# caishiqing/voice-tts

Measured on AMD Instinct MI355X. Metric: audio_seconds_per_second, higher is better.
Workload: dtype bf16

## Files before the change

include/ixtts_hip.h:

```cpp
#ifndef IXTTS_HIP_H
#define IXTTS_HIP_H

#include <stddef.h>
#include <stdint.h>

#ifdef __cplusplus
extern "C" {
#endif

#define IXTTS_OK 0
#define IXTTS_ERR_ARG (-1)
#define IXTTS_ERR_HIP (-2)
#define IXTTS_ERR_STATE (-3)
#define IXTTS_ERR_NOMEM (-4)
#define IXTTS_ERR_NAME (-5)

const char* ixtts_version(void);
const char* ixtts_last_error(void);

int ixtts_aa_snake_f32(const float* x_dev, float* y_dev, const float* up12_dev, const float* down12_dev,
                       const float* log_alpha_dev, const float* log_beta_dev, int B, int C, int T, void* stream);

size_t ixtts_attn_full_workspace_bytes(int B, int H, int T);
int ixtts_attn_full_f32(const float* q_dev, const float* k_dev, const float* v_dev, float* out_dev, int B, int H, int T,
// ... 18 lines not shown
int ixtts_adaln_rmsnorm_varlen_f32(const float* x_dev, const float* wb_dev, const float* g_dev, float* out_dev, const int* seq_off_dev, int nseq,
                                   long rows, int H, float eps, void* stream);
int ixtts_ln_modulate_varlen_f32(const float* x_dev, const float* shift_scale_dev, float* out_dev, const int* seq_off_dev, int nseq, long rows, int H,
                                 float eps, void* stream);
int ixtts_rope_qk_varlen_f32(float* qkv_dev, const float* cos_sin_dev, const int* seq_off_dev, int nseq, long rows, int H, int head_dim, void* stream);
int ixtts_wn_gate_rows_varlen_f32(const float* a_dev, const float* g_dev, float* out_dev, long rows, int C, const int* seq_off_dev, int nseq,
                                  long g_stride, int g_offset, void* stream);
int ixtts_reflect_halo_rows_varlen_f32(float* p_dev, const int* seq_off_dev, int nseq, int C, int left, int right, void* stream);

size_t ixtts_gemm_x6_packed_bytes(int N, int K);
int ixtts_gemm_x6_pack(const float* w_dev, void* packed_dev, int N, int K, void* stream);
long ixtts_gemm_x6_rows_padded(long rows);
int ixtts_gemm_x6_split(const float* a_dev, long lda, void* planes_dev, long rows, int K, void* stream);
int ixtts_gemm_x6_f32(const void* a_planes_dev, long rows_total, long row0, const void* packed_dev, const float* bias_dev, float* c_dev, long ldc,
                      int M, int N, int K, int accumulate, int tile, void* stream);
int ixtts_gemm_x6_pair_f32(const void* a_planes_dev, long rows_total, long row0, int taps, const void* packed_dev, const float* bias_dev,
                           const float* gate_dev, long gate_ld, long rows_per_batch, int nbatch, float* c_dev, long ldc, int M, int N, int K,
                           int epilogue, int tile, void* stream);
int ixtts_gemm_x6_pair_gate_varlen_f32(const void* a_planes_dev, long rows_total, long row0, int taps, const void* packed_dev, const float* bias_dev,
                                       const float* gate_dev, long gate_ld, const int* seq_off_dev, int nseq, float* c_dev, long ldc, int M, int N,
                                       int K, int tile, void* stream);

#define IXTTS_BIGVGAN_MAX_STAGES 8
#define IXTTS_BIGVGAN_MAX_RESK 4

typedef struct ixtts_bigvgan_cfg {
  int num_mels;
  int upsample_initial_channel;
  int n_stages;
  int upsample_rates[IXTTS_BIGVGAN_MAX_STAGES];
  int upsample_kernel_sizes[IXTTS_BIGVGAN_MAX_STAGES];
  int n_resblock_kernels;
  int resblock_kernel_sizes[IXTTS_BIGVGAN_MAX_RESK];
  int resblock_dilations[IXTTS_BIGVGAN_MAX_RESK][3];
  int max_frames;
  int fast_sin;
// ... 132 lines not shown
```

voice-tts_amd/_lib.py:

```python
import ctypes as C
import os

HERE = os.path.dirname(os.path.abspath(__file__))
LIB_PATH = os.environ.get("IXTTS_LIB") or os.path.join(HERE, "libixtts_hip.so")

MAX_STAGES = 8
MAX_RESK = 4


class BigVGANCfg(C.Structure):
    _fields_ = [
        ("num_mels", C.c_int), ("upsample_initial_channel", C.c_int), ("n_stages", C.c_int),
        ("upsample_rates", C.c_int * MAX_STAGES), ("upsample_kernel_sizes", C.c_int * MAX_STAGES),
        ("n_resblock_kernels", C.c_int), ("resblock_kernel_sizes", C.c_int * MAX_RESK),
        ("resblock_dilations", (C.c_int * 3) * MAX_RESK), ("max_frames", C.c_int), ("fast_sin", C.c_int),
    ]


class GptCfg(C.Structure):
    _fields_ = [
        ("model_dim", C.c_int), ("layers", C.c_int), ("heads", C.c_int), ("n_mel_codes", C.c_int),
        ("n_mel_pos", C.c_int), ("n_text_tokens", C.c_int), ("n_text_pos", C.c_int),
        ("start_mel_token", C.c_int), ("stop_mel_token", C.c_int), ("max_seq", C.c_int),
        ("max_batch", C.c_int), ("weight_dtype", C.c_int),
# ... 45 lines not shown
    "ixtts_reflect_halo_rows_f32": (C.c_int, [_P, C.c_int, C.c_int, C.c_int, C.c_int, C.c_int, _P]),
    "ixtts_adaln_rmsnorm_varlen_f32": (C.c_int, [_P, _P, _P, _P, _P, C.c_int, C.c_long, C.c_int, C.c_float, _P]),
    "ixtts_ln_modulate_varlen_f32": (C.c_int, [_P, _P, _P, _P, C.c_int, C.c_long, C.c_int, C.c_float, _P]),
    "ixtts_rope_qk_varlen_f32": (C.c_int, [_P, _P, _P, C.c_int, C.c_long, C.c_int, C.c_int, _P]),
    "ixtts_wn_gate_rows_varlen_f32": (C.c_int, [_P, _P, _P, C.c_long, C.c_int, _P, C.c_int, C.c_long, C.c_int, _P]),
    "ixtts_reflect_halo_rows_varlen_f32": (C.c_int, [_P, _P, C.c_int, C.c_int, C.c_int, C.c_int, _P]),
    "ixtts_gemm_x6_packed_bytes": (C.c_size_t, [C.c_int, C.c_int]),
    "ixtts_gemm_x6_pack": (C.c_int, [_P, _P, C.c_int, C.c_int, _P]),
    "ixtts_gemm_x6_rows_padded": (C.c_long, [C.c_long]),
    "ixtts_gemm_x6_split": (C.c_int, [_P, C.c_long, _P, C.c_long, C.c_int, _P]),
    "ixtts_gemm_x6_f32": (C.c_int, [_P, C.c_long, C.c_long, _P, _P, _P, C.c_long, C.c_int, C.c_int, C.c_int, C.c_int, C.c_int, _P]),
    "ixtts_gemm_x6_pair_f32": (C.c_int, [_P, C.c_long, C.c_long, C.c_int, _P, _P, _P, C.c_long, C.c_long, C.c_int, _P, C.c_long, C.c_int, C.c_int,
                                         C.c_int, C.c_int, C.c_int, _P]),
    "ixtts_gemm_x6_pair_gate_varlen_f32": (C.c_int, [_P, C.c_long, C.c_long, C.c_int, _P, _P, _P, C.c_long, _P, C.c_int, _P, C.c_long, C.c_int, C.c_int,
                                                     C.c_int, C.c_int, _P]),
    "ixtts_bigvgan_create": (C.c_int, [C.POINTER(_P), C.POINTER(BigVGANCfg)]),
    "ixtts_bigvgan_set_tensor": (C.c_int, [_P, C.c_char_p, _P, C.POINTER(C.c_int64), C.c_int]),
    "ixtts_bigvgan_finalize": (C.c_int, [_P]),
    "ixtts_bigvgan_arena": (C.c_int, [_P, C.POINTER(_P), C.POINTER(C.c_size_t)]),
    "ixtts_bigvgan_adopt_arena": (C.c_int, [_P]),
    "ixtts_bigvgan_forward": (C.c_int, [_P, _P, C.c_int, C.c_int, _P, _P]),
    "ixtts_bigvgan_flops": (C.c_double, [_P, C.c_int, C.c_int]),
    "ixtts_bigvgan_destroy": (C.c_int, [_P]),
    "ixtts_gpt_create": (C.c_int, [C.POINTER(_P), C.POINTER(GptCfg)]),
    "ixtts_gpt_set_tensor": (C.c_int, [_P, C.c_char_p, _P, C.POINTER(C.c_int64), C.c_int]),
    "ixtts_gpt_finalize": (C.c_int, [_P]),
    "ixtts_gpt_arena": (C.c_int, [_P, C.POINTER(_P), C.POINTER(C.c_size_t)]),
    "ixtts_gpt_adopt_arena": (C.c_int, [_P]),
    "ixtts_gpt_share_arena": (C.c_int, [_P, _P]),
    "ixtts_gpt_prefill": (C.c_int, [_P, C.c_int, _P, C.c_int, C.c_int, _P]),
# ... 74 lines not shown
```

voice-tts_amd/csrc/gemm_x6.hip:

```cpp
#include "common.h"

namespace ixtts {

typedef float gx_f32x16 __attribute__((ext_vector_type(16)));
typedef __bf16 gx_bf16x8 __attribute__((ext_vector_type(8)));
typedef float gx_f32x4 __attribute__((ext_vector_type(4)));
typedef unsigned int gx_u32x4 __attribute__((ext_vector_type(4)));


__global__ void gemm_x6_pack_kernel(const float* __restrict__ w, uint4* __restrict__ out, int N, int K, int Npad) {
  const long total = (long)(K / 8) * Npad;
  for (long idx = blockIdx.x * (long)blockDim.x + threadIdx.x; idx < total; idx += (long)gridDim.x * blockDim.x) {
    const int n = (int)(idx % Npad);
    const int ko = (int)(idx / Npad);
    float v[8];
#pragma unroll
    for (int e = 0; e < 8; ++e) v[e] = n < N ? w[(long)n * K + ko * 8 + e] : 0.f;
    uint4 ph, pm, pl;
    split8_bf16x3(v, ph, pm, pl);
    const int g = ko >> 1, kh = ko & 1;
    uint4* base = out + ((long)g * 6) * Npad + n;
    base[(long)(0 * 2 + kh) * Npad] = ph;
    base[(long)(1 * 2 + kh) * Npad] = pm;
    base[(long)(2 * 2 + kh) * Npad] = pl;
// ... 34 lines not shown
  const uint4* Ap;
  long Mpad;
  long arow0;
  const uint4* Wp;
  const float* bias;
  float* C;
  long ldc;
  int M, N, Npad, K, accumulate, m_tiles, n_tiles;
  int tap_steps;
  int epi;
  const float* gate;
  long gate_ld, rows_per_batch;
  int nbatch;
  const int* gate_seq_off;
  unsigned long long* dbg;
};


template <int MT, int NT, int NST, int DBG = 0>
__global__ __launch_bounds__(256, (NST * (MT + NT) * 6 * 64 * 16 <= 80 * 1024) ? 2 : 1) void gemm_x6_kernel(GemmX6Params p) {
  constexpr int BM = 64 * MT, BN = 64 * NT;
  constexpr int A_UNITS = 6 * BM, W_UNITS = 6 * BN, STAGE = A_UNITS + W_UNITS;
  constexpr int NDMA = (6 * (MT + NT)) / 4;
  static_assert((6 * (MT + NT)) % 4 == 0, "the copies are dealt evenly to the 4 waves");
  constexpr int D = NST - 1;
  extern __shared__ uint4 smem[];

  const int nwg = p.m_tiles * p.n_tiles;
  const int bid = blockIdx.x;
  const int xcd = bid & 7, idx = bid >> 3;
  const int qd = nwg >> 3, rm = nwg & 7;
  const int lin = (xcd < rm ? xcd * (qd + 1) : rm * (qd + 1) + (xcd - rm) * qd) + idx;
  const int m_tile = lin / p.n_tiles, n_tile = lin - m_tile * p.n_tiles;
  const int m0 = m_tile * BM, n0 = n_tile * BN;

  const int tid = threadIdx.x, lane = tid & 63, wave = tid >> 6;
  const int wm = wave >> 1, wn = wave & 1;
  const int l31 = lane & 31, lh = lane >> 5;

  gx_f32x16 acc[MT][NT];
#pragma unroll
  for (int i = 0; i < MT; ++i)
#pragma unroll
    for (int j = 0; j < NT; ++j)
#pragma unroll
      for (int r = 0; r < 16; ++r) acc[i][j][r] = 0.f;

// ... 4 lines not shown
#pragma unroll
    for (int q = 0; q < NDMA; ++q) {
      const int e = q * 4 + wave;
      if (e < 6 * MT) {
        const int run = e / MT, piece = e % MT;
        __builtin_amdgcn_global_load_lds((const __attribute__((address_space(1))) void*)(asrc + ((long)sa * 6 + run) * p.Mpad + tap + piece * 64),
                                         (__attribute__((address_space(3))) void*)(st + run * BM + piece * 64), 16, 0, 0);
      } else {
        const int e2 = e - 6 * MT, run = e2 / NT, piece = e2 % NT;
        __builtin_amdgcn_global_load_lds((const __attribute__((address_space(1))) void*)(wsrc + ((long)s * 6 + run) * p.Npad + piece * 64),
                                         (__attribute__((address_space(3))) void*)(st + A_UNITS + run * BN + piece * 64), 16, 0, 0);
      }
    }
  };

  const int steps = p.K >> 4;
  auto wg_stamp = [&](int k) {
    if constexpr (DBG == 3) {
      if (tid == 0) p.dbg[128 + (long)blockIdx.x * 4 + k] = __builtin_amdgcn_s_memrealtime();
    }
  };
  auto wait_younger = [&](int y) {
    if (y >= 2) asm volatile("s_waitcnt vmcnt(%0)" ::"n"(2 * NDMA) : "memory");
    else if (y == 1) asm volatile("s_waitcnt vmcnt(%0)" ::"n"(NDMA) : "memory");
    else asm volatile("s_waitcnt vmcnt(0)" ::: "memory");
  };
  static_assert(D >= 1 && D <= 3, "1..3 steps of copies in flight behind the one waited for");
  wg_stamp(0);
  for (int t = 0; t < D && t < steps; ++t) issue(t, smem + t * STAGE);
  wait_younger(min(D, steps) - 1);
  __builtin_amdgcn_s_barrier();
  asm volatile("" ::: "memory");
  wg_stamp(1);

  const unsigned base_addr = (unsigned)(uintptr_t)(const __attribute__((address_space(3))) void*)smem;
  int st_cur = 0, st_nxt = D % NST;
  for (int s = 0; s < steps; ++s) {
    auto stamp = [&](int k) {
      if constexpr (DBG == 3) {
        if (blockIdx.x == 0 && tid == 0 && s < 16) {
          p.dbg[s * 8 + k] = __builtin_amdgcn_s_memtime();
          if (k == 0) p.dbg[s * 8 + 7] = __builtin_amdgcn_s_memrealtime();
        }
      }
    };
    stamp(0);
    if (DBG != 1 && s + D < steps) issue(s + D, smem + st_nxt * STAGE);
    stamp(1);
    const unsigned cur_addr = base_addr + (unsigned)(st_cur * STAGE * 16);
    if constexpr (DBG != 2) {
      gx_u32x4 af[3][MT], bf[3][NT];
      const unsigned aaddr = cur_addr + (unsigned)((lh * BM + wm * (32 * MT) + l31) * 16);
      const unsigned waddr = cur_addr + (unsigned)((A_UNITS + lh * BN + wn * (32 * NT) + l31) * 16);
      if constexpr (MT == 4 && NT == 2) {
        asm volatile(
            "ds_read_b128 %0, %18 offset:%20\n ds_read_b128 %1, %18 offset:%21\n ds_read_b128 %2, %18 offset:%22\n ds_read_b128 %3, %18 offset:%23\n"
            "ds_read_b128 %4, %18 offset:%24\n ds_read_b128 %5, %18 offset:%25\n ds_read_b128 %6, %18 offset:%26\n ds_read_b128 %7, %18 offset:%27\n"
// ... 37 lines not shown
          acc[i][j] = __builtin_amdgcn_mfma_f32_32x32x16_bf16(ah, bh, acc[i][j], 0, 0, 0);
        }
      if constexpr (DBG == 3) asm volatile("" ::"v"(acc[0][0][0]), "v"(acc[MT - 1][NT - 1][15]));
    }
    stamp(3);
    wait_younger(DBG == 1 ? 0 : max(0, min(D - 1, steps - s - 2)));
    stamp(4);
    __builtin_amdgcn_s_barrier();
    asm volatile("" ::: "memory");
    stamp(5);
    st_cur = st_cur + 1 == NST ? 0 : st_cur + 1;
    st_nxt = st_nxt + 1 == NST ? 0 : st_nxt + 1;
  }

  wg_stamp(2);
  if (p.epi != EPI_PLAIN) {
    static_assert(NT == 2, "pair epilogues: the wave's two 32-column blocks are the two halves");
    const int oc = (n0 + wn * 64) / 2 + l31;
    const int nh = p.N >> 1;
    if (oc < nh) {
      const float ba = p.bias != nullptr ? p.bias[n0 + wn * 64 + l31] : 0.f, bb = p.bias != nullptr ? p.bias[n0 + wn * 64 + 32 + l31] : 0.f;
#pragma unroll
      for (int i = 0; i < MT; ++i) {
        const int rbase = m0 + wm * (32 * MT) + i * 32 + 4 * lh;
#pragma unroll
        for (int r = 0; r < 16; ++r) {
          const int row = rbase + (r & 3) + 8 * (r >> 2);
          if (row < p.M) {
            float a = acc[i][0][r] + ba, b = acc[i][1][r] + bb, v;
            if (p.epi == EPI_SWIGLU) {
// ... 25 lines not shown
        if (col_ok && row < p.M) {
          float* c = p.C + (long)row * p.ldc + col;
          float v = acc[i][j][r] + bv;
          if (p.accumulate) v += *c;
          *c = v;
        }
      }
    }
  }
  if constexpr (DBG == 3) {
    asm volatile("s_waitcnt vmcnt(0)" ::: "memory");
    wg_stamp(3);
  }
}

template <int MT, int NT, int NST, int DBG = 0>
static int launch_gemm_x6(GemmX6Params p, hipStream_t st) {
  constexpr int BM = 64 * MT, BN = 64 * NT;
  constexpr size_t smem = (size_t)NST * (6 * BM + 6 * BN) * 16;
  static_assert(smem <= 160 * 1024, "LDS stages of this tile shape");
  p.m_tiles = ceil_div(p.M, BM);
  p.n_tiles = ceil_div(p.N, BN);
  IX_ARG((long)p.n_tiles * BN <= p.Npad, "gemm_x6: packed weights padded to %d features, the %d-wide tile needs %d", p.Npad, BN, p.n_tiles * BN);
  const int taps = (p.K >> 4) / p.tap_steps;
  IX_ARG(p.arow0 + (long)p.m_tiles * BM + taps - 1 <= p.Mpad, "gemm_x6: activation planes hold %ld rows, the %d-row tiles reach row %ld", p.Mpad, BM,
         p.arow0 + (long)p.m_tiles * BM + taps - 1);
  auto kern = gemm_x6_kernel<MT, NT, NST, DBG>;
  static bool done = false;
  if (!done) {
    IX_HIP(hipFuncSetAttribute((const void*)kern, hipFuncAttributeMaxDynamicSharedMemorySize, (int)smem));
    done = true;
  }
  hipLaunchKernelGGL(kern, dim3(p.m_tiles * p.n_tiles), dim3(256), smem, st, p);
  IX_HIP(hipGetLastError());
  return IXTTS_OK;
}

}

using namespace ixtts;

extern "C" size_t ixtts_gemm_x6_packed_bytes(int N, int K) {
  if (N <= 0 || K <= 0 || K % 64) return 0;
  const size_t Npad = (size_t)(N + 255) / 256 * 256;
  return (size_t)(K / 16) * 6 * Npad * 16;
}

extern "C" int ixtts_gemm_x6_pack(const float* w_dev, void* packed_dev, int N, int K, void* stream) {
// ... 6 lines not shown
  return IXTTS_OK;
}

extern "C" long ixtts_gemm_x6_rows_padded(long rows) { return rows <= 0 ? 0 : (rows + 255) / 256 * 256 + 256; }

extern "C" int ixtts_gemm_x6_split(const float* a_dev, long lda, void* planes_dev, long rows, int K, void* stream) {
  IX_ARG(a_dev && planes_dev && rows > 0 && K > 0 && K % 64 == 0, "gemm_x6_split: bad argument (K must be a multiple of 64)");
  IX_ARG(lda >= K && lda % 4 == 0 && (reinterpret_cast<uintptr_t>(a_dev) & 15) == 0, "gemm_x6_split: rows must be 16-byte aligned (lda %ld)", lda);
  const long Mpad = ixtts_gemm_x6_rows_padded(rows);
  hipLaunchKernelGGL(gemm_x6_split_kernel, dim3((unsigned)(Mpad / 64), K / 64), dim3(256), 0, (hipStream_t)stream, a_dev, lda,
                     reinterpret_cast<uint4*>(planes_dev), (int)rows, K, Mpad);
  IX_HIP(hipGetLastError());
  return IXTTS_OK;
}

static int run_gemm_x6(GemmX6Params p, int tile, hipStream_t st) {
  if (tile == 0) {
    const long t42 = (long)ceil_div(p.M, 256) * ceil_div(p.N, 128);
    tile = t42 >= 140 ? 2 : 3;
  }
  switch (tile) {
    case 2: return launch_gemm_x6<4, 2, 2>(p, st);
    case 3: return launch_gemm_x6<2, 2, 3>(p, st);
    case 4: return launch_gemm_x6<4, 2, 4>(p, st);
    case 5: return launch_gemm_x6<2, 2, 4>(p, st);
    case 12: return launch_gemm_x6<4, 2, 2, 1>(p, st);
    case 22: return launch_gemm_x6<4, 2, 2, 2>(p, st);
    case 32: return launch_gemm_x6<4, 2, 2, 3>(p, st);
    case 33: return launch_gemm_x6<2, 2, 3, 3>(p, st);
  }
  set_error("gemm_x6: tile %d (0 auto; 2 / 3: 256x128 / 128x128, two workgroups per CU; 4 / 5: the same, one per CU with a 4-stage ring)", tile);
  return IXTTS_ERR_ARG;
}

extern "C" int ixtts_gemm_x6_f32(const void* a_planes_dev, long rows_total, long row0, const void* packed_dev, const float* bias_dev, float* c_dev,
                                 long ldc, int M, int N, int K, int accumulate, int tile, void* stream) {
  IX_ARG(a_planes_dev && packed_dev && c_dev && M > 0 && N > 0 && K > 0 && K % 64 == 0, "gemm_x6: bad argument (K must be a multiple of 64: the split pass works on 64-wide k blocks)");
  IX_ARG(ldc >= N && row0 >= 0 && row0 + M <= rows_total, "gemm_x6: rows [%ld, %ld) of %ld, ldc %ld", row0, row0 + M, rows_total, ldc);
  GemmX6Params p;
  p.Ap = reinterpret_cast<const uint4*>(a_planes_dev); p.Mpad = ixtts_gemm_x6_rows_padded(rows_total); p.arow0 = row0;
  p.Wp = reinterpret_cast<const uint4*>(packed_dev); p.bias = bias_dev; p.C = c_dev; p.ldc = ldc;
  p.M = M; p.N = N; p.Npad = (N + 255) / 256 * 256; p.K = K; p.accumulate = accumulate ? 1 : 0; p.m_tiles = p.n_tiles = 0;
  p.tap_steps = K >> 4; p.epi = EPI_PLAIN; p.gate = nullptr; p.gate_ld = 0; p.rows_per_batch = 1; p.nbatch = 1; p.gate_seq_off = nullptr;
  p.dbg = (tile == 32 || tile == 33) ? reinterpret_cast<unsigned long long*>(const_cast<float*>(bias_dev)) : nullptr;
  if (p.dbg) p.bias = nullptr;
  return run_gemm_x6(p, tile, (hipStream_t)stream);
}

extern "C" int ixtts_gemm_x6_pair_f32(const void* a_planes_dev, long rows_total, long row0, int taps, const void* packed_dev, const float* bias_dev,
                                      const float* gate_dev, long gate_ld, long rows_per_batch, int nbatch, float* c_dev, long ldc, int M, int N, int K,
                                      int epilogue, int tile, void* stream) {
  IX_ARG(a_planes_dev && packed_dev && c_dev && M > 0 && N > 0 && taps > 0 && K > 0, "gemm_x6_pair: bad argument");
  IX_ARG(K % taps == 0 && (K / taps) % 64 == 0 && N % 64 == 0, "gemm_x6_pair: K %d = %d taps of a multiple of 64, N %d a multiple of 64", K, taps, N);
  IX_ARG(epilogue == EPI_SWIGLU || (epilogue == EPI_GATE && gate_dev && rows_per_batch > 0 && nbatch > 0 && gate_ld >= N / 2),
         "gemm_x6_pair: epilogue %d (1 swiglu; 2 gate, with gate biases)", epilogue);
  IX_ARG(ldc >= N / 2 && row0 >= 0 && row0 + M + taps - 1 <= rows_total, "gemm_x6_pair: rows [%ld, %ld) + %d taps of %ld, ldc %ld", row0, row0 + M, taps,
         rows_total, ldc);
  IX_ARG(tile == 0 || tile == 2 || tile == 3, "gemm_x6_pair: tile %d (0 auto, 2, 3)", tile);
  GemmX6Params p;
  p.Ap = reinterpret_cast<const uint4*>(a_planes_dev); p.Mpad = ixtts_gemm_x6_rows_padded(rows_total); p.arow0 = row0;
  p.Wp = reinterpret_cast<const uint4*>(packed_dev); p.bias = bias_dev; p.C = c_dev; p.ldc = ldc;
  p.M = M; p.N = N; p.Npad = (N + 255) / 256 * 256; p.K = K; p.accumulate = 0; p.m_tiles = p.n_tiles = 0;
  p.tap_steps = (K / taps) >> 4; p.epi = epilogue; p.gate = gate_dev; p.gate_ld = gate_ld; p.rows_per_batch = rows_per_batch; p.nbatch = nbatch;
  p.gate_seq_off = nullptr;
  p.dbg = nullptr;
  return run_gemm_x6(p, tile, (hipStream_t)stream);
}

extern "C" int ixtts_gemm_x6_pair_gate_varlen_f32(const void* a_planes_dev, long rows_total, long row0, int taps, const void* packed_dev, const float* bias_dev,
                                                  const float* gate_dev, long gate_ld, const int* seq_off_dev, int nseq, float* c_dev, long ldc, int M, int N,
                                                  int K, int tile, void* stream) {
  IX_ARG(seq_off_dev && nseq > 0, "gemm_x6_pair_gate_varlen: null offsets table or nseq %d", nseq);
  IX_ARG(a_planes_dev && packed_dev && c_dev && gate_dev && M > 0 && N > 0 && taps > 0 && K > 0 && gate_ld >= N / 2, "gemm_x6_pair_gate_varlen: bad argument");
  IX_ARG(K % taps == 0 && (K / taps) % 64 == 0 && N % 64 == 0, "gemm_x6_pair_gate_varlen: K %d = %d taps of a multiple of 64, N %d a multiple of 64", K, taps, N);
  IX_ARG(ldc >= N / 2 && row0 >= 0 && row0 + M + taps - 1 <= rows_total, "gemm_x6_pair_gate_varlen: rows [%ld, %ld) + %d taps of %ld, ldc %ld", row0, row0 + M,
         taps, rows_total, ldc);
  IX_ARG(tile == 0 || tile == 2 || tile == 3, "gemm_x6_pair_gate_varlen: tile %d (0 auto, 2, 3)", tile);
  GemmX6Params p;
  p.Ap = reinterpret_cast<const uint4*>(a_planes_dev); p.Mpad = ixtts_gemm_x6_rows_padded(rows_total); p.arow0 = row0;
  p.Wp = reinterpret_cast<const uint4*>(packed_dev); p.bias = bias_dev; p.C = c_dev; p.ldc = ldc;
  p.M = M; p.N = N; p.Npad = (N + 255) / 256 * 256; p.K = K; p.accumulate = 0; p.m_tiles = p.n_tiles = 0;
  p.tap_steps = (K / taps) >> 4; p.epi = EPI_GATE; p.gate = gate_dev; p.gate_ld = gate_ld; p.rows_per_batch = 1; p.nbatch = nseq;
  p.gate_seq_off = seq_off_dev;
  p.dbg = nullptr;
  return run_gemm_x6(p, tile, (hipStream_t)stream);
}
```

voice-tts_amd/gemm.py:

```python
import ctypes as C

import torch

from . import _lib


class PackedLinear:

    __slots__ = ("N", "K", "packed", "bias")

    def __init__(self, weight, bias=None):
        assert weight.is_cuda and weight.dim() == 2 and weight.shape[1] % 64 == 0, tuple(weight.shape)
        w = weight.detach().to(torch.float32).contiguous()
        self.N, self.K = int(w.shape[0]), int(w.shape[1])
        nbytes = _lib.lib().ixtts_gemm_x6_packed_bytes(self.N, self.K)
        self.packed = torch.empty(nbytes, dtype=torch.uint8, device=w.device)
        with torch.cuda.device(w.device):
            _lib.check(_lib.lib().ixtts_gemm_x6_pack(w.data_ptr(), self.packed.data_ptr(), self.N, self.K, _lib.current_stream_ptr()), "ixtts_gemm_x6_pack")
            torch.cuda.current_stream().synchronize()
        self.bias = None if bias is None else bias.detach().to(w.device, torch.float32).contiguous()


class Planes:

    __slots__ = ("buf", "rows", "K")

    def __init__(self, buf, rows, K):
        self.buf, self.rows, self.K = buf, rows, K


_POOL = {}


def usable(x, K):
    return x.is_cuda and x.dtype == torch.float32 and K % 64 == 0 and x.shape[-1] == K and x.stride(-1) == 1 and x.data_ptr() % 16 == 0 and \
        (x.dim() == 1 or (x.stride(-2) % 4 == 0 and x.stride(-2) >= K))


def split(x, slot=0):
    K = int(x.shape[-1])
    if x.dim() != 2:
        x = x.reshape(-1, K) if x.is_contiguous() else x.contiguous().reshape(-1, K)
    rows, lda = int(x.shape[0]), int(x.stride(0))
    L = _lib.lib()
    nbytes = (K // 16) * 6 * int(L.ixtts_gemm_x6_rows_padded(rows)) * 16
    key = (x.device, nbytes, slot)
# ... 7 lines not shown

def linear(x, pl, out=None, accumulate=False, bias=True, tile=0, row0=0, rows=None, lead=None):
    K, N = pl.K, pl.N
    if not isinstance(x, Planes):
        lead = tuple(x.shape[:-1]) if lead is None else lead
        x = split(x)
    assert x.K == K, (x.K, K)
    M = (x.rows - row0) if rows is None else int(rows)
    if out is None:
        assert not accumulate
        out = torch.empty(*(lead if lead is not None else (M,)), N, dtype=torch.float32, device=pl.packed.device)
    assert out.shape[-1] == N and out.stride(-1) == 1 and out.numel() >= M * N
    ldc = int(out.stride(-2)) if out.dim() >= 2 else N
    b = pl.bias if (bias and pl.bias is not None) else None
    with torch.cuda.device(pl.packed.device):
        rc = _lib.lib().ixtts_gemm_x6_f32(x.buf.data_ptr(), x.rows, int(row0), pl.packed.data_ptr(), b.data_ptr() if b is not None else None, out.data_ptr(), ldc,
                                          M, N, K, 1 if accumulate else 0, int(tile), _lib.current_stream_ptr())
    _lib.check(rc, "ixtts_gemm_x6_f32")
    return out


SWIGLU, GATE = 1, 2


def interleave_halves(a, b):
    F = a.shape[0]
    assert b.shape == a.shape and F % 32 == 0, (tuple(a.shape), tuple(b.shape))
    return torch.stack([a.reshape(F // 32, 32, *a.shape[1:]), b.reshape(F // 32, 32, *b.shape[1:])], 1).reshape(2 * F, *a.shape[1:]).contiguous()


def pair_linear(x, pl, epilogue, taps=1, out=None, gate=None, gate_off=0, rows_per_batch=1, row0=0, rows=None, tile=0, seq_off=None):
    if not isinstance(x, Planes):
        x = split(x)
    assert pl.K == taps * x.K and pl.N % 64 == 0, (pl.K, taps, x.K, pl.N)
    M = (x.rows - row0 - (taps - 1)) if rows is None else int(rows)
    if out is None:
        out = torch.empty(M, pl.N // 2, dtype=torch.float32, device=pl.packed.device)
    assert out.shape[-1] == pl.N // 2 and out.stride(-1) == 1 and out.numel() >= M * (pl.N // 2)
    ldc = int(out.stride(-2)) if out.dim() >= 2 else pl.N // 2
    gp, gld, nb = None, 0, 1
    if epilogue == GATE:
        assert gate.is_contiguous() and gate.dim() == 2 and gate_off + pl.N <= gate.shape[1]
        gp, gld, nb = gate.data_ptr() + 4 * int(gate_off), int(gate.shape[1]), int(gate.shape[0])
    b = pl.bias
    if seq_off is not None:
        assert epilogue == GATE and seq_off.tab.is_cuda and gate.shape[0] >= seq_off.n
        with torch.cuda.device(pl.packed.device):
            rc = _lib.lib().ixtts_gemm_x6_pair_gate_varlen_f32(x.buf.data_ptr(), x.rows, int(row0), int(taps), pl.packed.data_ptr(),
                                                               b.data_ptr() if b is not None else None, gp, gld, seq_off.tab.data_ptr(), int(seq_off.n),
                                                               out.data_ptr(), ldc, M, pl.N, pl.K, int(tile), _lib.current_stream_ptr())
        _lib.check(rc, "ixtts_gemm_x6_pair_gate_varlen_f32")
        return out
    with torch.cuda.device(pl.packed.device):
        rc = _lib.lib().ixtts_gemm_x6_pair_f32(x.buf.data_ptr(), x.rows, int(row0), int(taps), pl.packed.data_ptr(), b.data_ptr() if b is not None else None,
                                               gp, gld, int(rows_per_batch), nb, out.data_ptr(), ldc, M, pl.N, pl.K, int(epilogue), int(tile),
                                               _lib.current_stream_ptr())
    _lib.check(rc, "ixtts_gemm_x6_pair_f32")
    return out
```

Baseline: 40.62.

## Add split-K variant of x6 GEMM with workspace reduction for small tile counts

Adds split-K instantiations of the x6 GEMM kernel: each output tile's K range is divided among 2 or 4 workgroups. Each writes its partial accumulators to a global slab, and the last arriving workgroup, found through an atomic ticket counter, sums the slices and runs the epilogue. Auto tile selection picks the 2-way split when the 128x128 tile count is small relative to the CU count and K is long, to fill the GPU better. The cost is extra global traffic for the partials, a per-stream zeroed workspace, and atomic and fence overhead.

```diff
diff --git a/include/ixtts_hip.h b/include/ixtts_hip.h
--- a/include/ixtts_hip.h
+++ b/include/ixtts_hip.h
@@ -56,12 +56,21 @@
 int ixtts_gemm_x6_split(const float* a_dev, long lda, void* planes_dev, long rows, int K, void* stream);
 int ixtts_gemm_x6_f32(const void* a_planes_dev, long rows_total, long row0, const void* packed_dev, const float* bias_dev, float* c_dev, long ldc,
                       int M, int N, int K, int accumulate, int tile, void* stream);
+size_t ixtts_gemm_x6_splitk_workspace_bytes(int M, int N, int K, int tile);
+int ixtts_gemm_x6_ws_f32(const void* a_planes_dev, long rows_total, long row0, const void* packed_dev, const float* bias_dev, float* c_dev, long ldc,
+                         int M, int N, int K, int accumulate, int tile, void* workspace_dev, size_t workspace_bytes, void* stream);
 int ixtts_gemm_x6_pair_f32(const void* a_planes_dev, long rows_total, long row0, int taps, const void* packed_dev, const float* bias_dev,
                            const float* gate_dev, long gate_ld, long rows_per_batch, int nbatch, float* c_dev, long ldc, int M, int N, int K,
                            int epilogue, int tile, void* stream);
+int ixtts_gemm_x6_pair_ws_f32(const void* a_planes_dev, long rows_total, long row0, int taps, const void* packed_dev, const float* bias_dev,
+                              const float* gate_dev, long gate_ld, long rows_per_batch, int nbatch, float* c_dev, long ldc, int M, int N, int K,
+                              int epilogue, int tile, void* workspace_dev, size_t workspace_bytes, void* stream);
 int ixtts_gemm_x6_pair_gate_varlen_f32(const void* a_planes_dev, long rows_total, long row0, int taps, const void* packed_dev, const float* bias_dev,
                                        const float* gate_dev, long gate_ld, const int* seq_off_dev, int nseq, float* c_dev, long ldc, int M, int N,
                                        int K, int tile, void* stream);
+int ixtts_gemm_x6_pair_gate_varlen_ws_f32(const void* a_planes_dev, long rows_total, long row0, int taps, const void* packed_dev, const float* bias_dev,
+                                          const float* gate_dev, long gate_ld, const int* seq_off_dev, int nseq, float* c_dev, long ldc, int M, int N,
+                                          int K, int tile, void* workspace_dev, size_t workspace_bytes, void* stream);
 
 #define IXTTS_BIGVGAN_MAX_STAGES 8
 #define IXTTS_BIGVGAN_MAX_RESK 4
diff --git a/voice-tts_amd/_lib.py b/voice-tts_amd/_lib.py
--- a/voice-tts_amd/_lib.py
+++ b/voice-tts_amd/_lib.py
@@ -83,6 +83,12 @@
                                          C.c_int, C.c_int, C.c_int, _P]),
     "ixtts_gemm_x6_pair_gate_varlen_f32": (C.c_int, [_P, C.c_long, C.c_long, C.c_int, _P, _P, _P, C.c_long, _P, C.c_int, _P, C.c_long, C.c_int, C.c_int,
                                                      C.c_int, C.c_int, _P]),
+    "ixtts_gemm_x6_splitk_workspace_bytes": (C.c_size_t, [C.c_int, C.c_int, C.c_int, C.c_int]),
+    "ixtts_gemm_x6_ws_f32": (C.c_int, [_P, C.c_long, C.c_long, _P, _P, _P, C.c_long, C.c_int, C.c_int, C.c_int, C.c_int, C.c_int, _P, C.c_size_t, _P]),
+    "ixtts_gemm_x6_pair_ws_f32": (C.c_int, [_P, C.c_long, C.c_long, C.c_int, _P, _P, _P, C.c_long, C.c_long, C.c_int, _P, C.c_long, C.c_int, C.c_int,
+                                            C.c_int, C.c_int, C.c_int, _P, C.c_size_t, _P]),
+    "ixtts_gemm_x6_pair_gate_varlen_ws_f32": (C.c_int, [_P, C.c_long, C.c_long, C.c_int, _P, _P, _P, C.c_long, _P, C.c_int, _P, C.c_long, C.c_int,
+                                                        C.c_int, C.c_int, C.c_int, _P, C.c_size_t, _P]),
     "ixtts_bigvgan_create": (C.c_int, [C.POINTER(_P), C.POINTER(BigVGANCfg)]),
     "ixtts_bigvgan_set_tensor": (C.c_int, [_P, C.c_char_p, _P, C.POINTER(C.c_int64), C.c_int]),
     "ixtts_bigvgan_finalize": (C.c_int, [_P]),
diff --git a/voice-tts_amd/csrc/gemm_x6.hip b/voice-tts_amd/csrc/gemm_x6.hip
--- a/voice-tts_amd/csrc/gemm_x6.hip
+++ b/voice-tts_amd/csrc/gemm_x6.hip
@@ -72,10 +72,15 @@
   int nbatch;
   const int* gate_seq_off;
   unsigned long long* dbg;
+  float4* ws_slab;
+  unsigned* ws_cnt;
 };
 
-
-template <int MT, int NT, int NST, int DBG = 0>
+constexpr int GX_SPLITK_MAX_TILES = 16384;
+constexpr size_t GX_SPLITK_CNT_BYTES = GX_SPLITK_MAX_TILES * 4;
+
+
+template <int MT, int NT, int NST, int DBG = 0, int SPLITK = 1>
 __global__ __launch_bounds__(256, (NST * (MT + NT) * 6 * 64 * 16 <= 80 * 1024) ? 2 : 1) void gemm_x6_kernel(GemmX6Params p) {
   constexpr int BM = 64 * MT, BN = 64 * NT;
   constexpr int A_UNITS = 6 * BM, W_UNITS = 6 * BN, STAGE = A_UNITS + W_UNITS;
@@ -84,11 +89,12 @@
   constexpr int D = NST - 1;
   extern __shared__ uint4 smem[];
 
-  const int nwg = p.m_tiles * p.n_tiles;
+  const int nwg = p.m_tiles * p.n_tiles * SPLITK;
   const int bid = blockIdx.x;
   const int xcd = bid & 7, idx = bid >> 3;
   const int qd = nwg >> 3, rm = nwg & 7;
-  const int lin = (xcd < rm ? xcd * (qd + 1) : rm * (qd + 1) + (xcd - rm) * qd) + idx;
+  const int lin_z = (xcd < rm ? xcd * (qd + 1) : rm * (qd + 1) + (xcd - rm) * qd) + idx;
+  const int lin = lin_z / SPLITK, zsl = lin_z - lin * SPLITK;
   const int m_tile = lin / p.n_tiles, n_tile = lin - m_tile * p.n_tiles;
   const int m0 = m_tile * BM, n0 = n_tile * BN;
 
@@ -123,7 +129,9 @@
     }
   };
 
-  const int steps = p.K >> 4;
+  const int steps_all = p.K >> 4;
+  const int s_lo = SPLITK > 1 ? (int)((long)zsl * steps_all / SPLITK) : 0;
+  const int steps = SPLITK > 1 ? (int)((long)(zsl + 1) * steps_all / SPLITK) : steps_all;
   auto wg_stamp = [&](int k) {
     if constexpr (DBG == 3) {
       if (tid == 0) p.dbg[128 + (long)blockIdx.x * 4 + k] = __builtin_amdgcn_s_memrealtime();
@@ -136,20 +144,20 @@
   };
   static_assert(D >= 1 && D <= 3, "1..3 steps of copies in flight behind the one waited for");
   wg_stamp(0);
-  for (int t = 0; t < D && t < steps; ++t) issue(t, smem + t * STAGE);
-  wait_younger(min(D, steps) - 1);
+  for (int t = 0; t < D && s_lo + t < steps; ++t) issue(s_lo + t, smem + t * STAGE);
+  wait_younger(min(D, steps - s_lo) - 1);
   __builtin_amdgcn_s_barrier();
   asm volatile("" ::: "memory");
   wg_stamp(1);
 
   const unsigned base_addr = (unsigned)(uintptr_t)(const __attribute__((address_space(3))) void*)smem;
   int st_cur = 0, st_nxt = D % NST;
-  for (int s = 0; s < steps; ++s) {
+  for (int s = s_lo; s < steps; ++s) {
     auto stamp = [&](int k) {
       if constexpr (DBG == 3) {
-        if (blockIdx.x == 0 && tid == 0 && s < 16) {
-          p.dbg[s * 8 + k] = __builtin_amdgcn_s_memtime();
-          if (k == 0) p.dbg[s * 8 + 7] = __builtin_amdgcn_s_memrealtime();
+        if (blockIdx.x == 0 && tid == 0 && s - s_lo < 16) {
+          p.dbg[(s - s_lo) * 8 + k] = __builtin_amdgcn_s_memtime();
+          if (k == 0) p.dbg[(s - s_lo) * 8 + 7] = __builtin_amdgcn_s_memrealtime();
         }
       }
     };
@@ -217,6 +225,70 @@
   }
 
   wg_stamp(2);
+  if constexpr (SPLITK > 1 && DBG != 4) {
+    constexpr int CH = MT * NT * 4;
+    float4* slab0 = p.ws_slab + ((long)lin * SPLITK) * (CH * 256) + tid;
+    {
+      float4* mine = slab0 + (long)zsl * (CH * 256);
+#pragma unroll
+      for (int i = 0; i < MT; ++i)
+#pragma unroll
+        for (int j = 0; j < NT; ++j)
+#pragma unroll
+          for (int c = 0; c < 4; ++c)
+            mine[((i * NT + j) * 4 + c) * 256] = make_float4(acc[i][j][4 * c], acc[i][j][4 * c + 1], acc[i][j][4 * c + 2], acc[i][j][4 * c + 3]);
+    }
+    asm volatile("s_waitcnt vmcnt(0)" ::: "memory");
+    __syncthreads();
+    volatile unsigned* last_flag = reinterpret_cast<volatile unsigned*>(smem);
+    if (tid == 0) {
+      __builtin_amdgcn_fence(__ATOMIC_RELEASE, "agent");
+      asm volatile("s_waitcnt vmcnt(0)" ::: "memory");
+      const unsigned ticket = __hip_atomic_fetch_add(p.ws_cnt + lin, 1u, __ATOMIC_RELAXED, __HIP_MEMORY_SCOPE_AGENT);
+      const bool last = ticket == SPLITK - 1;
+      if (last) {
+        __hip_atomic_store(p.ws_cnt + lin, 0u, __ATOMIC_RELAXED, __HIP_MEMORY_SCOPE_AGENT);
+        __builtin_amdgcn_fence(__ATOMIC_ACQUIRE, "agent");
+        asm volatile("s_waitcnt vmcnt(0)" ::: "memory");
+      }
+      *last_flag = last ? 1u : 0u;
+    }
+    __syncthreads();
+    if (*last_flag == 0u) {
+      wg_stamp(3);
+      return;
+    }
+    if constexpr (SPLITK == 2) {
+      const float4* other = slab0 + (long)(1 - zsl) * (CH * 256);
+#pragma unroll
+      for (int i = 0; i < MT; ++i)
+#pragma unroll
+        for (int j = 0; j < NT; ++j)
+#pragma unroll
+          for (int c = 0; c < 4; ++c) {
+            const float4 v = other[((i * NT + j) * 4 + c) * 256];
+            acc[i][j][4 * c] += v.x; acc[i][j][4 * c + 1] += v.y; acc[i][j][4 * c + 2] += v.z; acc[i][j][4 * c + 3] += v.w;
+          }
+    } else {
+#pragma unroll
+      for (int z = 0; z < SPLITK; ++z) {
+        const float4* sl = slab0 + (long)z * (CH * 256);
+#pragma unroll
+        for (int i = 0; i < MT; ++i)
+#pragma unroll
+          for (int j = 0; j < NT; ++j)
+#pragma unroll
+            for (int c = 0; c < 4; ++c) {
+              const float4 v = sl[((i * NT + j) * 4 + c) * 256];
+              if (z == 0) {
+                acc[i][j][4 * c] = v.x; acc[i][j][4 * c + 1] = v.y; acc[i][j][4 * c + 2] = v.z; acc[i][j][4 * c + 3] = v.w;
+              } else {
+                acc[i][j][4 * c] += v.x; acc[i][j][4 * c + 1] += v.y; acc[i][j][4 * c + 2] += v.z; acc[i][j][4 * c + 3] += v.w;
+              }
+            }
+      }
+    }
+  }
   if (p.epi != EPI_PLAIN) {
     static_assert(NT == 2, "pair epilogues: the wave's two 32-column blocks are the two halves");
     const int oc = (n0 + wn * 64) / 2 + l31;
@@ -272,7 +344,7 @@
   }
 }
 
-template <int MT, int NT, int NST, int DBG = 0>
+template <int MT, int NT, int NST, int DBG = 0, int SPLITK = 1>
 static int launch_gemm_x6(GemmX6Params p, hipStream_t st) {
   constexpr int BM = 64 * MT, BN = 64 * NT;
   constexpr size_t smem = (size_t)NST * (6 * BM + 6 * BN) * 16;
@@ -283,13 +355,17 @@
   const int taps = (p.K >> 4) / p.tap_steps;
   IX_ARG(p.arow0 + (long)p.m_tiles * BM + taps - 1 <= p.Mpad, "gemm_x6: activation planes hold %ld rows, the %d-row tiles reach row %ld", p.Mpad, BM,
          p.arow0 + (long)p.m_tiles * BM + taps - 1);
-  auto kern = gemm_x6_kernel<MT, NT, NST, DBG>;
+  if (SPLITK > 1) {
+    IX_ARG(p.ws_slab && p.ws_cnt, "gemm_x6: the split-K tile needs the workspace of ixtts_gemm_x6_splitk_workspace_bytes");
+    IX_ARG((long)p.m_tiles * p.n_tiles <= GX_SPLITK_MAX_TILES, "gemm_x6: split-K over %ld tiles (at most %d)", (long)p.m_tiles * p.n_tiles, GX_SPLITK_MAX_TILES);
+  }
+  auto kern = gemm_x6_kernel<MT, NT, NST, DBG, SPLITK>;
   static bool done = false;
   if (!done) {
     IX_HIP(hipFuncSetAttribute((const void*)kern, hipFuncAttributeMaxDynamicSharedMemorySize, (int)smem));
     done = true;
   }
-  hipLaunchKernelGGL(kern, dim3(p.m_tiles * p.n_tiles), dim3(256), smem, st, p);
+  hipLaunchKernelGGL(kern, dim3(p.m_tiles * p.n_tiles * SPLITK), dim3(256), smem, st, p);
   IX_HIP(hipGetLastError());
   return IXTTS_OK;
 }
@@ -326,27 +402,70 @@
   return IXTTS_OK;
 }
 
-static int run_gemm_x6(GemmX6Params p, int tile, hipStream_t st) {
+static int auto_tile(int M, int N, int K, bool may_split) {
+  const long t42 = (long)ceil_div(M, 256) * ceil_div(N, 128);
+  if (t42 >= 140) return 2;
+  const long t22 = (long)ceil_div(M, 128) * ceil_div(N, 128);
+  if (may_split && 2 * t22 < 3 * 256 && (K >> 4) >= 64) return 6;
+  return 3;
+}
+
+static int splitk_of_tile(int tile, int M, int N, long* tiles) {
+  switch (tile) {
+    case 6: case 36: case 46: *tiles = (long)ceil_div(M, 128) * ceil_div(N, 128); return 2;
+    case 7: *tiles = (long)ceil_div(M, 256) * ceil_div(N, 128); return 4;
+  }
+  *tiles = 0;
+  return 0;
+}
+
+extern "C" size_t ixtts_gemm_x6_splitk_workspace_bytes(int M, int N, int K, int tile) {
+  if (M <= 0 || N <= 0 || K <= 0) return 0;
+  if (tile == 0) tile = auto_tile(M, N, K, true);
+  long tiles = 0;
+  const int sk = splitk_of_tile(tile, M, N, &tiles);
+  if (sk == 0 || tiles > GX_SPLITK_MAX_TILES) return 0;
+  const size_t tile_bytes = (tile == 7 ? 256 : 128) * 128 * sizeof(float);
+  return GX_SPLITK_CNT_BYTES + (size_t)tiles * sk * tile_bytes;
+}
+
+static int run_gemm_x6(GemmX6Params p, int tile, void* ws, size_t ws_bytes, hipStream_t st) {
+  p.ws_slab = nullptr; p.ws_cnt = nullptr;
   if (tile == 0) {
-    const long t42 = (long)ceil_div(p.M, 256) * ceil_div(p.N, 128);
-    tile = t42 >= 140 ? 2 : 3;
+    const size_t need = ixtts_gemm_x6_splitk_workspace_bytes(p.M, p.N, p.K, 0);
+    tile = auto_tile(p.M, p.N, p.K, ws != nullptr && need != 0 && ws_bytes >= need);
+  }
+  {
+    long tiles = 0;
+    if (splitk_of_tile(tile, p.M, p.N, &tiles) != 0) {
+      const size_t need = ixtts_gemm_x6_splitk_workspace_bytes(p.M, p.N, p.K, tile);
+      IX_ARG(ws != nullptr && need != 0 && ws_bytes >= need && (reinterpret_cast<uintptr_t>(ws) & 15) == 0,
+             "gemm_x6: tile %d splits K and needs a 16-byte aligned workspace of %zu bytes (zeroed once), %zu given", tile, need, ws_bytes);
+      p.ws_cnt = reinterpret_cast<unsigned*>(ws);
+      p.ws_slab = reinterpret_cast<float4*>(reinterpret_cast<char*>(ws) + GX_SPLITK_CNT_BYTES);
+    }
   }
   switch (tile) {
     case 2: return launch_gemm_x6<4, 2, 2>(p, st);
     case 3: return launch_gemm_x6<2, 2, 3>(p, st);
     case 4: return launch_gemm_x6<4, 2, 4>(p, st);
     case 5: return launch_gemm_x6<2, 2, 4>(p, st);
+    case 6: return launch_gemm_x6<2, 2, 3, 0, 2>(p, st);
+    case 7: return launch_gemm_x6<4, 2, 2, 0, 4>(p, st);
     case 12: return launch_gemm_x6<4, 2, 2, 1>(p, st);
     case 22: return launch_gemm_x6<4, 2, 2, 2>(p, st);
     case 32: return launch_gemm_x6<4, 2, 2, 3>(p, st);
     case 33: return launch_gemm_x6<2, 2, 3, 3>(p, st);
-  }
-  set_error("gemm_x6: tile %d (0 auto; 2 / 3: 256x128 / 128x128, two workgroups per CU; 4 / 5: the same, one per CU with a 4-stage ring)", tile);
+    case 36: return launch_gemm_x6<2, 2, 3, 3, 2>(p, st);
+    case 46: return launch_gemm_x6<2, 2, 3, 4, 2>(p, st);
+  }
+  set_error("gemm_x6: tile %d (0 auto; 2 / 3: 256x128 / 128x128, two workgroups per CU; 4 / 5: the same, one per CU with a 4-stage ring; "
+            "6 / 7: 128x128 with K split in 2 / 256x128 with K split in 4)", tile);
   return IXTTS_ERR_ARG;
 }
 
-extern "C" int ixtts_gemm_x6_f32(const void* a_planes_dev, long rows_total, long row0, const void* packed_dev, const float* bias_dev, float* c_dev,
-                                 long ldc, int M, int N, int K, int accumulate, int tile, void* stream) {
+extern "C" int ixtts_gemm_x6_ws_f32(const void* a_planes_dev, long rows_total, long row0, const void* packed_dev, const float* bias_dev, float* c_dev,
+                                    long ldc, int M, int N, int K, int accumulate, int tile, void* workspace_dev, size_t workspace_bytes, void* stream) {
   IX_ARG(a_planes_dev && packed_dev && c_dev && M > 0 && N > 0 && K > 0 && K % 64 == 0, "gemm_x6: bad argument (K must be a multiple of 64: the split pass works on 64-wide k blocks)");
   IX_ARG(ldc >= N && row0 >= 0 && row0 + M <= rows_total, "gemm_x6: rows [%ld, %ld) of %ld, ldc %ld", row0, row0 + M, rows_total, ldc);
   GemmX6Params p;
@@ -354,21 +473,26 @@
   p.Wp = reinterpret_cast<const uint4*>(packed_dev); p.bias = bias_dev; p.C = c_dev; p.ldc = ldc;
   p.M = M; p.N = N; p.Npad = (N + 255) / 256 * 256; p.K = K; p.accumulate = accumulate ? 1 : 0; p.m_tiles = p.n_tiles = 0;
   p.tap_steps = K >> 4; p.epi = EPI_PLAIN; p.gate = nullptr; p.gate_ld = 0; p.rows_per_batch = 1; p.nbatch = 1; p.gate_seq_off = nullptr;
-  p.dbg = (tile == 32 || tile == 33) ? reinterpret_cast<unsigned long long*>(const_cast<float*>(bias_dev)) : nullptr;
+  p.dbg = (tile == 32 || tile == 33 || tile == 36) ? reinterpret_cast<unsigned long long*>(const_cast<float*>(bias_dev)) : nullptr;
   if (p.dbg) p.bias = nullptr;
-  return run_gemm_x6(p, tile, (hipStream_t)stream);
-}
-
-extern "C" int ixtts_gemm_x6_pair_f32(const void* a_planes_dev, long rows_total, long row0, int taps, const void* packed_dev, const float* bias_dev,
-                                      const float* gate_dev, long gate_ld, long rows_per_batch, int nbatch, float* c_dev, long ldc, int M, int N, int K,
-                                      int epilogue, int tile, void* stream) {
+  return run_gemm_x6(p, tile, workspace_dev, workspace_bytes, (hipStream_t)stream);
+}
+
+extern "C" int ixtts_gemm_x6_f32(const void* a_planes_dev, long rows_total, long row0, const void* packed_dev, const float* bias_dev, float* c_dev,
+                                 long ldc, int M, int N, int K, int accumulate, int tile, void* stream) {
+  return ixtts_gemm_x6_ws_f32(a_planes_dev, rows_total, row0, packed_dev, bias_dev, c_dev, ldc, M, N, K, accumulate, tile, nullptr, 0, stream);
+}
+
+extern "C" int ixtts_gemm_x6_pair_ws_f32(const void* a_planes_dev, long rows_total, long row0, int taps, const void* packed_dev, const float* bias_dev,
+                                         const float* gate_dev, long gate_ld, long rows_per_batch, int nbatch, float* c_dev, long ldc, int M, int N, int K,
+                                         int epilogue, int tile, void* workspace_dev, size_t workspace_bytes, void* stream) {
   IX_ARG(a_planes_dev && packed_dev && c_dev && M > 0 && N > 0 && taps > 0 && K > 0, "gemm_x6_pair: bad argument");
   IX_ARG(K % taps == 0 && (K / taps) % 64 == 0 && N % 64 == 0, "gemm_x6_pair: K %d = %d taps of a multiple of 64, N %d a multiple of 64", K, taps, N);
   IX_ARG(epilogue == EPI_SWIGLU || (epilogue == EPI_GATE && gate_dev && rows_per_batch > 0 && nbatch > 0 && gate_ld >= N / 2),
          "gemm_x6_pair: epilogue %d (1 swiglu; 2 gate, with gate biases)", epilogue);
   IX_ARG(ldc >= N / 2 && row0 >= 0 && row0 + M + taps - 1 <= rows_total, "gemm_x6_pair: rows [%ld, %ld) + %d taps of %ld, ldc %ld", row0, row0 + M, taps,
          rows_total, ldc);
-  IX_ARG(tile == 0 || tile == 2 || tile == 3, "gemm_x6_pair: tile %d (0 auto, 2, 3)", tile);
+  IX_ARG(tile == 0 || tile == 2 || tile == 3 || tile == 6 || tile == 7, "gemm_x6_pair: tile %d (0 auto, 2, 3, 6, 7)", tile);
   GemmX6Params p;
   p.Ap = reinterpret_cast<const uint4*>(a_planes_dev); p.Mpad = ixtts_gemm_x6_rows_padded(rows_total); p.arow0 = row0;
   p.Wp = reinterpret_cast<const uint4*>(packed_dev); p.bias = bias_dev; p.C = c_dev; p.ldc = ldc;
@@ -376,18 +500,25 @@
   p.tap_steps = (K / taps) >> 4; p.epi = epilogue; p.gate = gate_dev; p.gate_ld = gate_ld; p.rows_per_batch = rows_per_batch; p.nbatch = nbatch;
   p.gate_seq_off = nullptr;
   p.dbg = nullptr;
-  return run_gemm_x6(p, tile, (hipStream_t)stream);
-}
-
-extern "C" int ixtts_gemm_x6_pair_gate_varlen_f32(const void* a_planes_dev, long rows_total, long row0, int taps, const void* packed_dev, const float* bias_dev,
-                                                  const float* gate_dev, long gate_ld, const int* seq_off_dev, int nseq, float* c_dev, long ldc, int M, int N,
-                                                  int K, int tile, void* stream) {
+  return run_gemm_x6(p, tile, workspace_dev, workspace_bytes, (hipStream_t)stream);
+}
+
+extern "C" int ixtts_gemm_x6_pair_f32(const void* a_planes_dev, long rows_total, long row0, int taps, const void* packed_dev, const float* bias_dev,
+                                      const float* gate_dev, long gate_ld, long rows_per_batch, int nbatch, float* c_dev, long ldc, int M, int N, int K,
+                                      int epilogue, int tile, void* stream) {
+  return ixtts_gemm_x6_pair_ws_f32(a_planes_dev, rows_total, row0, taps, packed_dev, bias_dev, gate_dev, gate_ld, rows_per_batch, nbatch, c_dev, ldc, M, N, K,
+                                   epilogue, tile, nullptr, 0, stream);
+}
+
+extern "C" int ixtts_gemm_x6_pair_gate_varlen_ws_f32(const void* a_planes_dev, long rows_total, long row0, int taps, const void* packed_dev,
+                                                     const float* bias_dev, const float* gate_dev, long gate_ld, const int* seq_off_dev, int nseq, float* c_dev,
+                                                     long ldc, int M, int N, int K, int tile, void* workspace_dev, size_t workspace_bytes, void* stream) {
   IX_ARG(seq_off_dev && nseq > 0, "gemm_x6_pair_gate_varlen: null offsets table or nseq %d", nseq);
   IX_ARG(a_planes_dev && packed_dev && c_dev && gate_dev && M > 0 && N > 0 && taps > 0 && K > 0 && gate_ld >= N / 2, "gemm_x6_pair_gate_varlen: bad argument");
   IX_ARG(K % taps == 0 && (K / taps) % 64 == 0 && N % 64 == 0, "gemm_x6_pair_gate_varlen: K %d = %d taps of a multiple of 64, N %d a multiple of 64", K, taps, N);
   IX_ARG(ldc >= N / 2 && row0 >= 0 && row0 + M + taps - 1 <= rows_total, "gemm_x6_pair_gate_varlen: rows [%ld, %ld) + %d taps of %ld, ldc %ld", row0, row0 + M,
          taps, rows_total, ldc);
-  IX_ARG(tile == 0 || tile == 2 || tile == 3, "gemm_x6_pair_gate_varlen: tile %d (0 auto, 2, 3)", tile);
+  IX_ARG(tile == 0 || tile == 2 || tile == 3 || tile == 6 || tile == 7, "gemm_x6_pair_gate_varlen: tile %d (0 auto, 2, 3, 6, 7)", tile);
   GemmX6Params p;
   p.Ap = reinterpret_cast<const uint4*>(a_planes_dev); p.Mpad = ixtts_gemm_x6_rows_padded(rows_total); p.arow0 = row0;
   p.Wp = reinterpret_cast<const uint4*>(packed_dev); p.bias = bias_dev; p.C = c_dev; p.ldc = ldc;
@@ -395,5 +526,12 @@
   p.tap_steps = (K / taps) >> 4; p.epi = EPI_GATE; p.gate = gate_dev; p.gate_ld = gate_ld; p.rows_per_batch = 1; p.nbatch = nseq;
   p.gate_seq_off = seq_off_dev;
   p.dbg = nullptr;
-  return run_gemm_x6(p, tile, (hipStream_t)stream);
-}
+  return run_gemm_x6(p, tile, workspace_dev, workspace_bytes, (hipStream_t)stream);
+}
+
+extern "C" int ixtts_gemm_x6_pair_gate_varlen_f32(const void* a_planes_dev, long rows_total, long row0, int taps, const void* packed_dev, const float* bias_dev,
+                                                  const float* gate_dev, long gate_ld, const int* seq_off_dev, int nseq, float* c_dev, long ldc, int M, int N,
+                                                  int K, int tile, void* stream) {
+  return ixtts_gemm_x6_pair_gate_varlen_ws_f32(a_planes_dev, rows_total, row0, taps, packed_dev, bias_dev, gate_dev, gate_ld, seq_off_dev, nseq, c_dev, ldc, M,
+                                               N, K, tile, nullptr, 0, stream);
+}
diff --git a/voice-tts_amd/gemm.py b/voice-tts_amd/gemm.py
--- a/voice-tts_amd/gemm.py
+++ b/voice-tts_amd/gemm.py
@@ -1,4 +1,5 @@
 import ctypes as C
+import os
 
 import torch
 
@@ -30,6 +31,27 @@
 
 
 _POOL = {}
+
+
+_SPLITK_WS = {}
+
+
+def splitk_bytes(M, N, K, tile=0):
+    if tile == 0 and os.environ.get("IXTTS_S2MEL_GEMM") == "x6_nosplit":
+        return 0
+    return int(_lib.lib().ixtts_gemm_x6_splitk_workspace_bytes(int(M), int(N), int(K), int(tile)))
+
+
+def _splitk_ws(device, M, N, K, tile):
+    need = splitk_bytes(M, N, K, tile)
+    if need == 0:
+        return None, 0
+    key = (device, int(torch.cuda.current_stream(device).cuda_stream))
+    ws = _SPLITK_WS.get(key)
+    if ws is None or ws.numel() < need:
+        with torch.cuda.device(device):
+            ws = _SPLITK_WS[key] = torch.zeros(need, dtype=torch.uint8, device=device)
+    return ws.data_ptr(), ws.numel()
 
 
 def usable(x, K):
@@ -67,9 +89,10 @@
     ldc = int(out.stride(-2)) if out.dim() >= 2 else N
     b = pl.bias if (bias and pl.bias is not None) else None
     with torch.cuda.device(pl.packed.device):
-        rc = _lib.lib().ixtts_gemm_x6_f32(x.buf.data_ptr(), x.rows, int(row0), pl.packed.data_ptr(), b.data_ptr() if b is not None else None, out.data_ptr(), ldc,
-                                          M, N, K, 1 if accumulate else 0, int(tile), _lib.current_stream_ptr())
-    _lib.check(rc, "ixtts_gemm_x6_f32")
+        wsp, wsn = _splitk_ws(pl.packed.device, M, N, K, tile)
+        rc = _lib.lib().ixtts_gemm_x6_ws_f32(x.buf.data_ptr(), x.rows, int(row0), pl.packed.data_ptr(), b.data_ptr() if b is not None else None, out.data_ptr(),
+                                             ldc, M, N, K, 1 if accumulate else 0, int(tile), wsp, wsn, _lib.current_stream_ptr())
+    _lib.check(rc, "ixtts_gemm_x6_ws_f32")
     return out
 
 
@@ -99,14 +122,16 @@
     if seq_off is not None:
         assert epilogue == GATE and seq_off.tab.is_cuda and gate.shape[0] >= seq_off.n
         with torch.cuda.device(pl.packed.device):
-            rc = _lib.lib().ixtts_gemm_x6_pair_gate_varlen_f32(x.buf.data_ptr(), x.rows, int(row0), int(taps), pl.packed.data_ptr(),
-                                                               b.data_ptr() if b is not None else None, gp, gld, seq_off.tab.data_ptr(), int(seq_off.n),
-                                                               out.data_ptr(), ldc, M, pl.N, pl.K, int(tile), _lib.current_stream_ptr())
-        _lib.check(rc, "ixtts_gemm_x6_pair_gate_varlen_f32")
+            wsp, wsn = _splitk_ws(pl.packed.device, M, pl.N, pl.K, tile)
+            rc = _lib.lib().ixtts_gemm_x6_pair_gate_varlen_ws_f32(x.buf.data_ptr(), x.rows, int(row0), int(taps), pl.packed.data_ptr(),
+                                                                  b.data_ptr() if b is not None else None, gp, gld, seq_off.tab.data_ptr(), int(seq_off.n),
+                                                                  out.data_ptr(), ldc, M, pl.N, pl.K, int(tile), wsp, wsn, _lib.current_stream_ptr())
+        _lib.check(rc, "ixtts_gemm_x6_pair_gate_varlen_ws_f32")
         return out
     with torch.cuda.device(pl.packed.device):
-        rc = _lib.lib().ixtts_gemm_x6_pair_f32(x.buf.data_ptr(), x.rows, int(row0), int(taps), pl.packed.data_ptr(), b.data_ptr() if b is not None else None,
-                                               gp, gld, int(rows_per_batch), nb, out.data_ptr(), ldc, M, pl.N, pl.K, int(epilogue), int(tile),
-                                               _lib.current_stream_ptr())
-    _lib.check(rc, "ixtts_gemm_x6_pair_f32")
+        wsp, wsn = _splitk_ws(pl.packed.device, M, pl.N, pl.K, tile)
+        rc = _lib.lib().ixtts_gemm_x6_pair_ws_f32(x.buf.data_ptr(), x.rows, int(row0), int(taps), pl.packed.data_ptr(), b.data_ptr() if b is not None else None,
+                                                  gp, gld, int(rows_per_batch), nb, out.data_ptr(), ldc, M, pl.N, pl.K, int(epilogue), int(tile), wsp, wsn,
+                                                  _lib.current_stream_ptr())
+    _lib.check(rc, "ixtts_gemm_x6_pair_ws_f32")
     return out
```

Result: no change. 40.72, median of 2 (+0.2%).
